# cfframe/spatial-VAE

Hardware: AMD Instinct MI355X
Metric: images/sec (ELBO fwd+bwd+step), MNIST 28x28 batch=256, 1/2/4/8 GPU (higher is better)
Workload: dtype f32; 1 GPU; mnist-rotated-translated 28x28 z=2 H=500x2 tanh B=256 (BASELINE configs[1]); global_batch=256, per_gpu_batch=256, pixels=784, parallelism=dp1

## Files before the change

### spatial_vae_amd/csrc/api.hip

```cpp
#include <stdarg.h>
#include <stdio.h>
#include <stdlib.h>
#include <string.h>
#include <math.h>
#include <atomic>
#include <mutex>
#include <iterator>
#include <type_traits>
#include <unordered_map>
#include <vector>

#include "common.h"
#include "../../include/svae_stream.h"
#include "../../include/svae_align.h"
#include "../../include/svae_ctfcorr.h"
#include "../../include/svae_cluster.h"
#include "../../include/svae_frc.h"
#include "../../include/svae_refine.h"
#include "../../include/svae_classify.h"
#include "../../include/svae_gmm.h"
#include "../../include/svae_pca.h"
#include "../../include/svae_expect.h"
#include <hip/hip_ext.h>
#include "dense.h"
// ... 347 lines not shown
int launch_status(const char* what) {
    const hipError_t e = hipGetLastError();
    if (e != hipSuccess) return fail(SVAE_E_LAUNCH, "%s: %s", what, hipGetErrorString(e));
    return SVAE_OK;
}

inline unsigned blocks_for(long n) { return (unsigned)((n + 255) / 256); }

PoseArgs pose_args(const svae_pose* pose) {
    PoseArgs pa;
    pa.coords = pose->coords;
    pa.grid = pose->grid;
    pa.theta = pose->coords ? nullptr : pose->theta;
    pa.dx = pose->coords ? nullptr : pose->dx;
    return pa;
}

RowGeo row_geo(const Geo& g) {
    RowGeo r;
    r.N = g.N; r.Npad = g.Npad; r.Hp = g.Hp; r.in_dim = g.in_dim; r.act = g.act; r.B = g.B;
    return r;
}

void launch_prepare(const Geo& g, const Plan& pl, const svae_params* p, const PoseArgs& pa, const float* z, hipStream_t st) {
    Scope prof(K_PREPARE, st);
    PrepareArgs a;
    a.coord_w = p->coord_w; a.coord_b = p->coord_b;
    a.latent_w = g.Zd > 0 ? p->latent_w : nullptr;
    a.bil_w = (g.flags & SVAE_FLAG_BILINEAR) ? p->bilinear_w : nullptr;
    a.z = z; a.tab = pl.tab; a.posebuf = pl.posebuf; a.pose = pa;
    a.B = g.B; a.H = g.H; a.Hp = g.Hp; a.Zd = g.Zd; a.in_dim = g.in_dim;
    const long nt = (long)g.B * g.Hp;
    a.nb_tab = (int)blocks_for(nt > g.B ? nt : g.B);
    a.nb_pack = (int)blocks_for((long)g.Hp * g.Hp);
    a.nlayers = g.L - 1;
    for (int l = 0; l < SVAE_MAX_HIDDEN; ++l) {
        const bool on = l + 1 < g.L;
        a.W[l] = on ? p->hidden_w[l] : nullptr;
        a.wf[l] = on ? pl.wf[l] : nullptr;
        a.wb[l] = on ? pl.wb[l] : nullptr;
        a.wb_row_scale[l] = (on && l == g.L - 2 && rank1_out(g)) ? p->out_w : nullptr;
    }
    hipLaunchKernelGGL(prepare_kernel, dim3((unsigned)(a.nb_tab + a.nb_pack * a.nlayers)), dim3(256), 0, st, a);
}

template <int NT, bool DGRAD, bool RESID, bool FIRST, int LASTD, int CF = 0>
void launch_dense_ntr(const DenseArgs& a, dim3 grid, hipStream_t st) {
    constexpr int kLds = DenseCfg<NT>::LDS_BYTES + (LASTD == 1 ? SVAE_MAX_OUT * 4096 * 4 : 0);
    const int lds = DenseCfg<NT>::LDS_BYTES + (LASTD == 1 ? SVAE_MAX_OUT * a.Hp * 4 : 0);
    static bool attr_set = false;
    if (!attr_set) {
        (void)hipFuncSetAttribute(reinterpret_cast<const void*>(&dense_kernel<NT, DGRAD, RESID, FIRST, LASTD, CF>),
                                  hipFuncAttributeMaxDynamicSharedMemorySize, kLds < 160 * 1024 ? kLds : 160 * 1024);
        attr_set = true;
    }
    launch_gemm(dense_kernel<NT, DGRAD, RESID, FIRST, LASTD, CF>, grid, dim3(256), (unsigned)lds, st, a);
}

template <int NT, bool DGRAD>
void launch_dense_nt(const DenseArgs& a, dim3 grid, hipStream_t st, bool first = false, int lastd = 0, int cf = 0) {
    if constexpr (!DGRAD && NT <= 4) {
        if (cf >= 1) {
            if (a.resid) launch_dense_ntr<NT, false, true, false, 0, 1>(a, grid, st);
            else launch_dense_ntr<NT, false, false, false, 0, 1>(a, grid, st);
            return;
// ... 372 lines not shown
        else launch_gemm(wgrad2_kernel<0>, grid, dim3(256), 0u, st, w);
        return;
    }
    const int nb2 = w.nblk1 * w.nblk1;
    w.S = (xcd && nb2 > 1 && nsplit % 8 == 0) ? nsplit : 0;
    const dim3 grid = w.S ? dim3(nb2 * nsplit) : dim3(nb2, nsplit);
    if (r1 == 1) {
        launch_wgrad_c<1, 1>(w, grid, st);
        return;
    }
    if (r1 == 2) {
        launch_wgrad_c<1, 2>(w, grid, st);
        return;
    }
    switch (cl) {
        case 1: launch_wgrad_c<1>(w, grid, st); break;
        case 2: launch_wgrad_c<2>(w, grid, st); break;
        case 3: launch_wgrad_c<3>(w, grid, st); break;
        case 4: launch_wgrad_c<4>(w, grid, st); break;
        default: launch_wgrad_c<0>(w, grid, st); break;
    }
}

template <int ACT>
void launch_layer0_fwd(const Geo& g, const Plan& pl, const PoseArgs& pa, float* a0, hipStream_t st) {
    Scope prof(K_LAYER0_FWD, st);
    const int oimg = g.Npad / 8;
    const int cpi = (oimg + kL0Chunk - 1) / kL0Chunk;
    const int opc = (oimg + cpi - 1) / cpi;
    const long nchunks = (long)g.B * cpi;
    const unsigned gy = (unsigned)(nchunks < 32768 ? nchunks : 32768);
    const unsigned gz = (unsigned)((nchunks + gy - 1) / gy);
    hipLaunchKernelGGL((layer0_fwd_kernel<ACT>), dim3(blocks_for(g.Hp * 2), gy, gz), dim3(256), 0, st, pa, pl.posebuf,
                       pl.tab, a0, row_geo(g), opc, (oimg + opc - 1) / opc, nchunks);
}

template <int ACT>
void launch_layer0_fwd_split(const Geo& g, const Plan& pl, const PoseArgs& pa, float* a0, bool saved_ok, hipStream_t st) {
    Scope prof(K_LAYER0_FWD, st);
    hipLaunchKernelGGL((layer0_fwd_split_kernel<ACT>), dim3((unsigned)g.tiles, (unsigned)(g.Hp / 64)), dim3(256), 0, st, pa,
                       pl.posebuf, pl.tab, split_a0_fragments_only(g) ? (float*)nullptr : a0, pl.splitA,
                       (saved_ok && g.L == 2) ? pl.savedC : (uint4*)nullptr, row_geo(g));
}

template <int C>
void launch_out_fwd(const Geo& g, const float* a, const svae_params* p, float* y, float* logits, hipStream_t st) {
    Scope prof(K_OUT_FWD, st);
    long nb = (g.noct + 3) / 4;
    if (nb > 4096) nb = 4096;
    hipLaunchKernelGGL((out_fwd_kernel<C>), dim3((unsigned)nb), dim3(256), 0, st, a, p->out_w, p->out_b, y, logits,
                       row_geo(g), g.H, (g.flags & SVAE_FLAG_SOFTPLUS) ? 1 : 0, g.noct);
}

template <int ACT, int C>
void launch_out_bwd_ac(const Geo& g, const Plan& pl, const float* a, const svae_params* p, float* dh, hipStream_t st) {
    Scope prof(K_OUT_BWD, st);
    hipLaunchKernelGGL((out_bwd_kernel<ACT, C>), dim3(blocks_for(g.Hp * 2), pl.ob_chunks), dim3(256), 0, st, a, pl.do_p,
// ... 41 lines not shown
        return fail(SVAE_E_INVALID, "softplus output with a Bernoulli likelihood: the reference's binary_cross_entropy rejects "
                                    "values above 1 (train_mnist.py:81)");
    if (d->Zd > 0 && !z) return fail(SVAE_E_INVALID, "latent_dim > 0 but z is null");
    if (saved && (reinterpret_cast<uintptr_t>(saved) & 255)) return fail(SVAE_E_WORKSPACE, "saved not 256-byte aligned");
    const Geo g = make_geo(*d);
    Plan pl = make_plan(g, saved, ws);
    if ((rc = check_ws(pl, ws, ws_bytes))) return rc;
    hipStream_t st = static_cast<hipStream_t>(stream);
    const PoseArgs pa = pose_args(pose);
    if (!saved) {
        for (int l = 0; l < g.L; ++l) pl.act[l] = pl.dh[l & 1];
    } else {
        remember_plan(saved, plan_bits(g));
    }

    const char* fuse_e = getenv("SVAE_FUSE_LOGITS");
    const bool fuse_env = !(fuse_e && fuse_e[0] == '0');
    const bool split_fwd = split_mode() && (g.act == SVAE_ACT_TANH || g.act == SVAE_ACT_SIGMOID) && g.ntile % 2 == 0;
    const bool fuse_logits = fuse_env && g.L >= 2 &&
                             (split_fwd ? g.C <= 2
                                        : g.C <= 2 * (use_dense4(g, g.flags & SVAE_FLAG_RESID, 0) ? use_dense4(g, g.flags & SVAE_FLAG_RESID, 0)
                                                                                                   : dense_nt_first(g.ntile)));

    launch_prepare(g, pl, p, pa, z, st);
    const bool split = split_mode() && (g.act == SVAE_ACT_TANH || g.act == SVAE_ACT_SIGMOID) && g.ntile % 2 == 0;
    const bool split_l0 = split_l0_on() && split && g.L >= 2;
    if (split_l0) {
        if (g.act == SVAE_ACT_TANH) launch_layer0_fwd_split<SVAE_ACT_TANH>(g, pl, pa, pl.act[0], saved != nullptr, st);
        else launch_layer0_fwd_split<SVAE_ACT_SIGMOID>(g, pl, pa, pl.act[0], saved != nullptr, st);
    } else {
        switch (g.act) {
            case SVAE_ACT_TANH: launch_layer0_fwd<SVAE_ACT_TANH>(g, pl, pa, pl.act[0], st); break;
            case SVAE_ACT_LEAKYRELU: launch_layer0_fwd<SVAE_ACT_LEAKYRELU>(g, pl, pa, pl.act[0], st); break;
            case SVAE_ACT_RELU: launch_layer0_fwd<SVAE_ACT_RELU>(g, pl, pa, pl.act[0], st); break;
            default: launch_layer0_fwd<SVAE_ACT_SIGMOID>(g, pl, pa, pl.act[0], st); break;
        }
    }
    DenseBlocks cfb{dense_nt_first(g.ntile), (long)g.Mp, 1};
    for (int l = 1; l < g.L; ++l) {
        if (split) {
            launch_split_fwd(g, pl, pl.act[l - 1], p->hidden_w[l - 1], p->hidden_b[l - 1], pl.act[l],
                             (g.flags & SVAE_FLAG_RESID) != 0, (fuse_logits && l == g.L - 1) ? g.C : 0, p->out_w,
                             split_l0 && l == 1, st);
            continue;
        }
        DenseArgs a;
        a.in = pl.act[l - 1];
        a.wp = pl.wf[l - 1];
        a.out = pl.act[l];
        a.bias = p->hidden_b[l - 1];
        a.aux = nullptr;
        a.tiles = g.tiles;
        a.Hp = g.Hp;
        a.H = g.H;
        a.act = g.act;
        a.resid = (g.flags & SVAE_FLAG_RESID) ? 1 : 0;
        a.pose = pa; a.posebuf = nullptr; a.tab = nullptr; a.sgtile = nullptr; a.dfpart = nullptr;
        a.Mp = g.Mp; a.N = g.N; a.Timg = g.Timg;
        a.do_p = nullptr; a.out_w = p->out_w; a.C = g.C;
        a.lpart = pl.dfpart;
        const DenseBlocks used = launch_dense<false>(g, a, st, false, 0, (fuse_logits && l == g.L - 1) ? g.C : 0);
        if (l == g.L - 1) cfb = used;
    }
    if (fuse_logits) {
        Scope prof(K_OUT_FWD, st);
        const int nblk = g.ntile / (split ? split_nt_fwd(g) : cfb.nt);
        const long m_split = split ? (long)g.Mp : cfb.m_split;
        const int nblk_tail = g.ntile / cfb.nt_tail;
        if (bce_target) {
            const int chunks = finish_chunks(g.N);
            hipLaunchKernelGGL(logits_finish_bce_kernel, dim3(g.B, chunks), dim3(g.N > 512 ? 1024 : (g.N > 256 ? 512 : 256)), 0, st,
                               pl.dfpart, p->out_b, bce_target, y, logits, chunks > 1 ? pl.llpart : loglik, dll_dy, row_geo(g), g.C,
                               nblk, (long)g.Mp, m_split, nblk_tail);
            if (chunks > 1)
                hipLaunchKernelGGL(loglik_reduce_kernel, dim3(blocks_for(g.B)), dim3(256), 0, st, pl.llpart, loglik, g.B, chunks);
        }
        else
            hipLaunchKernelGGL(logits_finish_kernel, dim3(blocks_for((long)g.B * g.N)), dim3(256), 0, st, pl.dfpart, p->out_b, y,
                               logits, row_geo(g), g.C, nblk, (g.flags & SVAE_FLAG_SOFTPLUS) ? 1 : 0, (long)g.Mp, m_split, nblk_tail);
        return launch_status("svae_decoder_forward");
    }
    switch (g.C) {
// ... 32 lines not shown
    if ((rc = check_desc(d)) || (rc = check_params(d, p)) || (rc = check_pose(pose))) return rc;
    if (!logits || !dy || !saved || !grads) return fail(SVAE_E_INVALID, "logits, dy, saved and grads are required");
    if (d->Zd > 0 && !z) return fail(SVAE_E_INVALID, "latent_dim > 0 but z is null");
    if (reinterpret_cast<uintptr_t>(saved) & 255) return fail(SVAE_E_WORKSPACE, "saved not 256-byte aligned");
    if (pg && (pg->dtheta || pg->ddx) && pose->coords)
        return fail(SVAE_E_INVALID, "dtheta/ddx requested but the pose was given as explicit coords");
    const Geo g = make_geo(*d);
    {
        const long rec = recorded_plan(saved);
        if (rec >= 0 && (unsigned)rec != plan_bits(g))
            return fail(SVAE_E_INVALID, "svae_decoder_backward: `saved` was written by a forward call planned differently (plan "
                        "bits %ld then, %u now): the GEMM mode (svae_gemm_mode_set / SVAE_GEMM) or SVAE_FUSE_OUT changed between "
                        "the forward call and its backward call", rec, plan_bits(g));
    }
    const Plan pl = make_plan(g, const_cast<void*>(saved), ws);
    if ((rc = check_ws(pl, ws, ws_bytes))) return rc;
    hipStream_t st = static_cast<hipStream_t>(stream);
    const PoseArgs pa = pose_args(pose);
    const int resid = (g.flags & SVAE_FLAG_RESID) ? 1 : 0;
    const int fmode = fuse_out_mode();
    const bool split_bwd = split_active(g) && g.L >= 2 && fmode != 1;
    const bool r1 = rank1_out(g);

    {
        Scope prof(K_DLOGITS, st);
        if (split_bwd && hipMemsetAsync(pl.amax, 0, sizeof(unsigned), st) != hipSuccess) return fail(SVAE_E_LAUNCH, "memset failed");
        hipLaunchKernelGGL(dlogits_kernel, dim3(blocks_for((long)g.C * g.Mp)), dim3(256), 0, st, logits, dy, dy_scale,
                           pl.do_p, g.B, g.N, g.Npad, g.C, (g.flags & SVAE_FLAG_SOFTPLUS) ? 1 : 0, (long)g.Mp,
                           split_bwd ? pl.amax : (unsigned*)nullptr);
        if (split_bwd)
            hipLaunchKernelGGL(split_scale_kernel, dim3(1), dim3(256), 0, st, pl.amax, p->out_w, g.C, g.H, pl.gscale);
    }

    int cur = 0;
    const bool fused_out = r1 || (fmode == 1 && g.L >= 2 && !resid && (grads->hidden_w[g.L - 2] || grads->hidden_b[g.L - 2]));
    int ob_nparts = 0;
    static const bool ob_env = [] { const char* e = getenv("SVAE_SPLIT_OB"); return !(e && e[0] == '0'); }();
    const bool split_ob = ob_env && split_bwd && split_wgrad_on() && (grads->hidden_w[g.L - 2] || grads->hidden_b[g.L - 2]);
    if (split_ob) {
        const float* alast = pl.act[g.L - 1];
        float* dh32 = resid ? pl.dh[cur] : nullptr;
        const int nparts = g.act == SVAE_ACT_TANH ? launch_out_bwd_split_a<SVAE_ACT_TANH>(g, pl, alast, p, dh32, st)
                                                  : launch_out_bwd_split_a<SVAE_ACT_SIGMOID>(g, pl, alast, p, dh32, st);
        ob_nparts = nparts;
        Scope prof(K_SMALL_BWD, st);
        hipLaunchKernelGGL(out_bwd_reduce_kernel, dim3(g.C * ((g.Hp + 63) / 64) + 1), dim3(1024), 0, st, pl.wpart, pl.bpart,
                           grads->out_w, grads->out_b, g.C, g.H, g.Hp, nparts);
    } else if (!fused_out) {
        const float* alast = pl.act[g.L - 1];
        switch (g.act) {
            case SVAE_ACT_TANH: launch_out_bwd_a<SVAE_ACT_TANH>(g, pl, alast, p, pl.dh[cur], st); break;
            case SVAE_ACT_LEAKYRELU: launch_out_bwd_a<SVAE_ACT_LEAKYRELU>(g, pl, alast, p, pl.dh[cur], st); break;
            case SVAE_ACT_RELU: launch_out_bwd_a<SVAE_ACT_RELU>(g, pl, alast, p, pl.dh[cur], st); break;
            default: launch_out_bwd_a<SVAE_ACT_SIGMOID>(g, pl, alast, p, pl.dh[cur], st); break;
        }
        Scope prof(K_SMALL_BWD, st);
        hipLaunchKernelGGL(out_bwd_reduce_kernel, dim3(g.C * ((g.Hp + 63) / 64) + 1), dim3(1024), 0, st, pl.wpart, pl.bpart,
                           grads->out_w, grads->out_b, g.C, g.H, g.Hp, pl.ob_chunks * 2);
    }

    bool fused_first = false;
    bool tail_pending = false;
    WgradReduceArgs tail_r{};
    bool obr_pending = false;
    OutBwdReduceArgs tail_o{};
    const bool dcoords_wanted = pg && pg->dcoords;
    DenseBlocks fb{dense_nt_first(g.ntile), (long)g.Mp, 1};
    for (int l = g.L - 1; l >= 1; --l) {
        const bool last = fused_out && l == g.L - 1;
        const bool split_here = split_bwd && (l == g.L - 1 || split_chain_on());
        if (grads->hidden_w[l - 1] || grads->hidden_b[l - 1] || (last && (grads->out_w || grads->out_b))) {
            WgradArgs w;
            w.dh = last ? pl.act[l] : pl.dh[cur];
            w.aprev = pl.act[l - 1];
            w.slab = pl.slab;
            w.bslab = pl.bslab;
            w.noct = g.noct;
            w.vo = (g.N + 7) / 8; w.po = g.Npad / 8;
            w.Hp = g.Hp;
            w.nblk1 = pl.wg_nblk1;
            w.do_p = pl.do_p; w.out_w = p->out_w; w.wpart = pl.wpart; w.bpart = pl.bpart;
            w.Mp = g.Mp; w.H = g.H; w.act = g.act;
            if (split_here && split_wgrad_on())
                launch_split_wgrad(g, pl, pl.dh[cur], pl.act[l - 1],
                                   (l == 1 && g.L == 2 && split_l0_on()) ? pl.savedC : (const uint4*)nullptr,
                                   split_ob && l == g.L - 1, st);
            else {
                static const bool xcd_grid = [] { const char* e = getenv("SVAE_XCD_GRID"); return !(e && e[0] == '0'); }();
                launch_wgrad(w, pl.wg_S, xcd_grid, last ? g.C : 0, (last && r1) ? (g.act == SVAE_ACT_TANH ? 1 : 2) : 0, st);
            }
            Scope prof(K_WGRAD_REDUCE, st);
            const bool db_elsewhere = split_ob && l == g.L - 1 && split_wgrad_on();
            const WgradReduceArgs ra{pl.slab, pl.bslab, grads->hidden_w[l - 1],
                                     db_elsewhere ? (float*)nullptr : grads->hidden_b[l - 1], g.H, g.Hp, pl.wg_S,
                                     (last && r1) ? p->out_w : (const float*)nullptr};
            if (l == 1 && g.in_dim == 2 && !split_here && tail_merge_on()) {
                tail_r = ra;
                tail_pending = true;
            } else {
                hipLaunchKernelGGL(wgrad_reduce_kernel, dim3((unsigned)(((long)g.H * g.H + 63) / 64)), dim3(256), 0, st, ra);
            }
            if (db_elsewhere && grads->hidden_b[l - 1])
                hipLaunchKernelGGL(colsum_reduce_kernel, dim3(g.Hp / 32), dim3(256), 0, st, pl.hbpart, grads->hidden_b[l - 1],
                                   g.H, g.Hp, ob_nparts);
            if (last) {
                tail_o = OutBwdReduceArgs{pl.wpart, pl.bpart, grads->out_w, grads->out_b, g.C, g.H, g.Hp, pl.wg_S * 2};
                obr_pending = true;
            }
        }
        DenseArgs a;
        a.in = last ? pl.act[l] : pl.dh[cur];
        a.wp = pl.wb[l - 1];
        a.out = pl.dh[cur ^ 1];
        a.bias = nullptr;
        a.aux = pl.act[l - 1];
        a.tiles = g.tiles;
        a.Hp = g.Hp;
        a.H = g.H;
        a.act = g.act;
        a.resid = resid;
        a.pose = pa; a.posebuf = pl.posebuf; a.tab = pl.tab; a.sgtile = pl.sgtile; a.dfpart = pl.dfpart;
        a.Mp = g.Mp; a.N = g.N; a.Timg = g.Timg;
        a.do_p = pl.do_p; a.out_w = p->out_w; a.C = g.C;
        fused_first = (l == 1) && g.in_dim == 2;
        if (split_here)
            launch_split_dgrad(g, pl, pl.dh[cur], p->hidden_w[l - 1], pl.act[l - 1], pl.dh[cur ^ 1], resid != 0, fused_first, pa,
                               split_ob && l == g.L - 1, st);
        else {
            const DenseBlocks used = launch_dense<true>(g, a, st, fused_first, last ? (r1 ? (g.act == SVAE_ACT_TANH ? 2 : 3) : 1) : 0,
                                                        0, dcoords_wanted);
            if (l == 1) fb = used;
        }
        cur ^= 1;
    }

    if (tail_pending && !fused_first) {
        tail_pending = false;
        hipLaunchKernelGGL(wgrad_reduce_kernel, dim3((unsigned)(((long)g.H * g.H + 63) / 64)), dim3(256), 0, st, tail_r);
    }
    const unsigned obr_blocks = (unsigned)(g.C * ((g.Hp + 63) / 64) + 1);
    if (obr_pending && !tail_pending) {
        obr_pending = false;
        Scope prof(K_SMALL_BWD, st);
        hipLaunchKernelGGL(out_bwd_reduce_kernel, dim3(obr_blocks), dim3(1024), 0, st, tail_o.wpart, tail_o.bpart, tail_o.dWo,
                           tail_o.dbo, tail_o.C, tail_o.H, tail_o.Hp, tail_o.nparts);
    }
    const bool bil = (g.flags & SVAE_FLAG_BILINEAR) != 0;
    const bool want_coords = pg && (pg->dcoords || pg->dtheta || pg->ddx);
    float* dc = (pg && pg->dcoords) ? pg->dcoords : pl.dcoords;
    {
        Scope prof_l0(K_LAYER0_BWD, st);
        const bool split_first = split_bwd && (g.L == 2 || split_chain_on());
        const bool want_dz = dz && g.Zd > 0;
        const bool pose_sums = fused_first && !pose->coords && !dcoords_wanted && pg && (pg->dtheta || pg->ddx);
// ... 473 lines not shown
```

### spatial_vae_amd/csrc/common.h

```cpp
#pragma once
#include <hip/hip_runtime.h>
#include <stdint.h>

#include "../../include/svae.h"

namespace svae {

typedef float f32x16 __attribute__((ext_vector_type(16)));
typedef float v4f __attribute__((ext_vector_type(4)));

constexpr int kSlots = 8;
constexpr int kBiasSlot = 5;

struct Geo {
    int B, N, H, L, Zd, C, in_dim, act, flags;
    int Timg;
    int Npad;
    int Mp;
    int Hp;
    int ntile;
    long noct;
    long tiles;
};

// ... 67 lines not shown
    if (p.coords) {
        const float2 v = *reinterpret_cast<const float2*>(p.coords + ((long)b * N + i) * 2);
        return v;
    }
    const float2 g = *reinterpret_cast<const float2*>(p.grid + (long)i * 2);
    return make_float2(c * g.x - s * g.y + dx0, s * g.x + c * g.y + dx1);
}

__device__ __forceinline__ void image_pose(const PoseArgs& p, int b, float& c, float& s, float& dx0, float& dx1) {
    c = 1.0f; s = 0.0f; dx0 = 0.0f; dx1 = 0.0f;
    if (!p.coords) {
        if (p.theta) {
            const float t = p.theta[b];
            c = cosf(t);
            s = sinf(t);
        }
        if (p.dx) {
            dx0 = p.dx[2 * b];
            dx1 = p.dx[2 * b + 1];
        }
    }
}

__device__ __forceinline__ float2 row_coord(const PoseArgs& pose, const float4 pb, int b, int i, int N) {
    if (i >= N) return make_float2(0.0f, 0.0f);
    return pixel_coord(pose, b, i, N, pb.x, pb.y, pb.z, pb.w);
}

__device__ __forceinline__ void coord_feats(float2 x, float f[5]) {
    f[0] = x.x; f[1] = x.y; f[2] = x.x * x.x; f[3] = x.y * x.y; f[4] = x.x * x.y;
}

__device__ __forceinline__ float wave_sum32(float v) {
    v += __shfl_xor(v, 1);
    v += __shfl_xor(v, 2);
    v += __shfl_xor(v, 4);
    v += __shfl_xor(v, 8);
    v += __shfl_xor(v, 16);
    return v;
}

template <int CTRL, int ROW_MASK>
__device__ __forceinline__ float dpp_add(float v) {
    const int t = __builtin_amdgcn_update_dpp(0, __float_as_int(v), CTRL, ROW_MASK, 0xf, ROW_MASK == 0xf);
    return v + __int_as_float(t);
}
// ... 62 lines not shown
```

### spatial_vae_amd/csrc/dense.h

```cpp
#pragma once
#include "common.h"

namespace svae {

struct DenseArgs {
    const float* in;
    const float* wp;
    float* out;
    const float* bias;
    const float* aux;
    long tiles;
    int Hp;
    int H;
    int act;
    int resid;
    PoseArgs pose;
    const float4* posebuf;
    const float* tab;
    float* sgtile;
    float* dfpart;
    long Mp;
    int N, Timg;
    const float* do_p;
    const float* out_w;
    int C;
    float* lpart;
};

template <int ACT, bool DGRAD>
__device__ __forceinline__ float4 dense_epilogue(float4 v, float bias, float4 aux) {
    if (DGRAD) {
        v.x *= act_grad<ACT>(aux.x); v.y *= act_grad<ACT>(aux.y);
        v.z *= act_grad<ACT>(aux.z); v.w *= act_grad<ACT>(aux.w);
    } else {
        v.x = act_fwd<ACT>(v.x + bias); v.y = act_fwd<ACT>(v.y + bias);
        v.z = act_fwd<ACT>(v.z + bias); v.w = act_fwd<ACT>(v.w + bias);
    }
    return v;
}

__device__ __forceinline__ void glds16(const float* gsrc, unsigned lds_byte_addr) {
    unsigned keep;
    asm volatile(
        "s_mov_b32 %0, m0\n\ts_mov_b32 m0, %2\n\ts_nop 0\n\tglobal_load_lds_dwordx4 %1, off\n\ts_mov_b32 m0, %0"
        : "=&s"(keep)
        : "v"(gsrc), "s"(lds_byte_addr)
        : "memory");
}
__device__ __forceinline__ void dma_wait_all() { asm volatile("s_waitcnt vmcnt(0)" ::: "memory"); }
// ... 749 lines not shown
```

### spatial_vae_amd/csrc/dense4.h

```cpp
#pragma once
#include "dense.h"

namespace svae {

typedef float f32x4v __attribute__((ext_vector_type(4)));
typedef float f32x2v __attribute__((ext_vector_type(2)));

template <int OFF>
__device__ __forceinline__ void load_a4(const float* p, f32x4v& v) {
    asm volatile("global_load_dwordx4 %0, %1, off offset:%2" : "+v"(v) : "v"(p), "i"(OFF) : "memory");
}
template <int N>
__device__ __forceinline__ void wait_vm4(f32x4v& v) {
    asm volatile("s_waitcnt vmcnt(%1)" : "+v"(v) : "i"(N) : "memory");
}
template <int LASTD>
__device__ __forceinline__ f32x4v rank1_actgrad(f32x4v x) {
    f32x4v r;
#pragma unroll
    for (int i = 0; i < 4; ++i) r[i] = __builtin_fmaf(-x[i], x[i], LASTD == 2 ? 1.0f : x[i]);
    return r;
}

__device__ __forceinline__ float add_uncontracted(float a, float b) {
// ... 63 lines not shown
    auto read_b = [&](int o, float4 (&b)[NT]) {
        const float* base = bfrag + ((o / G) & 1) * CHUNK + (o % G) * NT * 256;
#pragma unroll
        for (int t = 0; t < NT; ++t) b[t] = *reinterpret_cast<const float4*>(base + t * 256);
    };
    constexpr int P = PW;
    constexpr int PE = (P + 3) / 4;
    static_assert(G == 4, "the slot offsets assume 4 octets per chunk");

    float* rowx = smem + 2 * CHUNK + wave * (3 * 128);
    if (FIRST) {
#pragma unroll
        for (int rr = 0; rr < 2; ++rr) {
            const int row = lane + 64 * rr;
            const long tile = rgl * 4 + (row >> 5);
            const int b = (int)(tile / a.Timg);
            const int i = (int)(tile % a.Timg) * 32 + (row & 31);
            const float4 pb = a.posebuf[b];
            const float* cbase = a.pose.coords ? a.pose.coords + (long)b * a.N * 2 : a.pose.grid;
            const float2 g2 = *reinterpret_cast<const float2*>(cbase + (long)(i < a.N ? i : a.N - 1) * 2);
            const bool in = i < a.N;
            rowx[row] = in ? pb.x * g2.x - pb.y * g2.y + pb.z : 0.0f;
            rowx[128 + row] = in ? pb.y * g2.x + pb.x * g2.y + pb.w : 0.0f;
            if (LASTD != 0) rowx[256 + row] = a.do_p[rgl * 128 + row];
        }
    }
    stage(0, 0);
    stage(nchunk > 1 ? 1 : 0, 1);
    f32x4v av[G][4];
    float4 b0[NT], b1[NT];
#pragma unroll
    for (int gl = 0; gl < G; ++gl)
#pragma unroll
        for (int e = 0; e < 4; ++e) av[gl][e] = f32x4v{0.0f, 0.0f, 0.0f, 0.0f};
    load_a4<0>(arow, av[0][0]); load_a4<32>(arow, av[0][1]); load_a4<64>(arow, av[0][2]); load_a4<96>(arow, av[0][3]);
    load_a4<256>(arow, av[1][0]); load_a4<288>(arow, av[1][1]); load_a4<320>(arow, av[1][2]); load_a4<352>(arow, av[1][3]);
    load_a4<512>(arow, av[2][0]); load_a4<544>(arow, av[2][1]); load_a4<576>(arow, av[2][2]); load_a4<608>(arow, av[2][3]);
    load_a4<768>(arow, av[3][0]); load_a4<800>(arow, av[3][1]); load_a4<832>(arow, av[3][2]); load_a4<864>(arow, av[3][3]);
#pragma unroll
    for (int gl = 0; gl < G; ++gl)
#pragma unroll
        for (int e = 0; e < 4; ++e) wait_vm4<0>(av[gl][e]);
    __syncthreads();
    read_b(0, b0);
    const int spare = nchunk & 1;
    auto kstep = [&](const f32x4v& x, const float4 (&bf)[NT], int e) {
#pragma unroll
// ... 266 lines not shown
```

### spatial_vae_amd/csrc/elementwise.h

```cpp
#pragma once
#include <type_traits>
#include "common.h"

namespace svae {

__device__ __forceinline__ long slab_index(int contr, int out, int ntile) {
    return (((long)(contr >> 3) * ntile + (out >> 5)) * 2 + ((contr >> 2) & 1)) * 128 + (out & 31) * 4 + (contr & 3);
}
struct PrepareArgs {
    const float* coord_w; const float* coord_b; const float* latent_w; const float* bil_w; const float* z;
    float* tab; float4* posebuf; PoseArgs pose;
    int B, H, Hp, Zd, in_dim;
    int nb_tab, nb_pack, nlayers;
    const float* W[SVAE_MAX_HIDDEN]; float* wf[SVAE_MAX_HIDDEN]; float* wb[SVAE_MAX_HIDDEN];
    const float* wb_row_scale[SVAE_MAX_HIDDEN];
};
__global__ void __launch_bounds__(256) prepare_kernel(PrepareArgs a) {
    if ((int)blockIdx.x < a.nb_tab) {
        const long idx = (long)blockIdx.x * 256 + threadIdx.x;
        if (idx < a.B) {
            float c, s, d0, d1;
            image_pose(a.pose, (int)idx, c, s, d0, d1);
            a.posebuf[idx] = make_float4(c, s, d0, d1);
        }
        if (idx >= (long)a.B * a.Hp) return;
        const int b = idx / a.Hp, k = idx % a.Hp;
        float out[kSlots] = {0, 0, 0, 0, 0, 0, 0, 0};
        if (k < a.H) {
            for (int p = 0; p < a.in_dim; ++p) {
                float w = a.coord_w[k * a.in_dim + p];
                if (a.bil_w)
                    for (int q = 0; q < a.Zd; ++q) w += a.bil_w[((long)k * a.in_dim + p) * a.Zd + q] * a.z[(long)b * a.Zd + q];
                out[p] = w;
            }
            float bias = a.coord_b[k];
            if (a.latent_w)
                for (int q = 0; q < a.Zd; ++q) bias += a.latent_w[(long)k * a.Zd + q] * a.z[(long)b * a.Zd + q];
            out[kBiasSlot] = bias;
        }
        float4* dst = reinterpret_cast<float4*>(a.tab + idx * kSlots);
        dst[0] = make_float4(out[0], out[1], out[2], out[3]);
        dst[1] = make_float4(out[4], out[5], out[6], out[7]);
        return;
    }
    const int rel = blockIdx.x - a.nb_tab;
    const int l = rel / a.nb_pack;
    const long idx = (long)(rel - l * a.nb_pack) * 256 + threadIdx.x;
    if (l >= a.nlayers || idx >= (long)a.Hp * a.Hp) return;
    const int n = idx / a.Hp, k = idx % a.Hp;
    const float v = (n < a.H && k < a.H) ? a.W[l][(long)n * a.H + k] : 0.0f;
    a.wf[l][slab_index(k, n, a.Hp / 32)] = v;
    a.wb[l][slab_index(n, k, a.Hp / 32)] = (a.wb_row_scale[l] && n < a.H) ? v * a.wb_row_scale[l][n] : v;
}

struct RowGeo {
    int N, Npad, Hp, in_dim, act, B;
};

constexpr int kL0Chunk = 32;
template <int ACT>
__global__ void __launch_bounds__(256) layer0_fwd_kernel(PoseArgs pose, const float4* __restrict__ posebuf,
                                                         const float* __restrict__ tab, float* __restrict__ a0, RowGeo g,
                                                         int oct_per_chunk, int chunks_per_image, long nchunks) {
    __shared__ float4 xs[kL0Chunk * 2 * 2];
    const long chunk = (long)blockIdx.z * gridDim.y + blockIdx.y;
    if (chunk >= nchunks) return;
    const int b = (int)(chunk / chunks_per_image), ci = (int)(chunk - (long)b * chunks_per_image);
    const int oimg = g.Npad >> 3;
    const int oc0 = ci * oct_per_chunk;
    const int noc = (oc0 + oct_per_chunk <= oimg) ? oct_per_chunk : oimg - oc0;
    const float4 pb = posebuf[b];
    const float* cbase = pose.coords ? pose.coords + (long)b * g.N * 2 : pose.grid;
    float* xf = reinterpret_cast<float*>(xs);
    for (int j = threadIdx.x; j < noc * 8; j += 256) {
        const int i = oc0 * 8 + j;
        float x0 = 0.0f, x1 = 0.0f;
        if (i < g.N) {
            const float2 raw = *reinterpret_cast<const float2*>(cbase + (long)i * 2);
            x0 = pb.x * raw.x - pb.y * raw.y + pb.z;
            x1 = pb.y * raw.x + pb.x * raw.y + pb.w;
        }
        const int slot = (j >> 2) * 8 + (j & 3);
        xf[slot] = x0;
        xf[slot + 4] = x1;
    }
    __syncthreads();
    const int t = blockIdx.x * 256 + threadIdx.x;
    if (t >= g.Hp * 2) return;
    const int h = t & 1, k = t >> 1;
    const float4* tp = reinterpret_cast<const float4*>(tab + ((long)b * g.Hp + k) * kSlots);
    const float4 t0 = tp[0], t1 = tp[1];
    const long ostride = (long)g.Hp * 8;
    float* dst = a0 + (((long)b * oimg + oc0) * g.Hp * 2 + t) * 4;
    const bool expand = g.in_dim == 5;
#pragma unroll 4
    for (int jo = 0; jo < noc; ++jo) {
        const float4 X0 = xs[(jo * 2 + h) * 2], X1 = xs[(jo * 2 + h) * 2 + 1];
        const float x0[4] = {X0.x, X0.y, X0.z, X0.w}, x1[4] = {X1.x, X1.y, X1.z, X1.w};
        float out[4];
#pragma unroll
        for (int e = 0; e < 4; ++e) {
            float v = t1.y + x0[e] * t0.x + x1[e] * t0.y;
            if (expand) v += (x0[e] * x0[e]) * t0.z + (x1[e] * x1[e]) * t0.w + (x0[e] * x1[e]) * t1.x;
            out[e] = act_fwd<ACT>(v);
        }
        *reinterpret_cast<float4*>(dst + jo * ostride) = make_float4(out[0], out[1], out[2], out[3]);
    }
}

template <int C>
__global__ void out_fwd_kernel(const float* __restrict__ a, const float* __restrict__ out_w,
                               const float* __restrict__ out_b, float* __restrict__ y, float* __restrict__ logits,
                               RowGeo g, int H, int softplus, long noct) {
    const int lane = threadIdx.x & 63;
    const int nl = lane & 31, h = lane >> 5;
    const long wave0 = (long)blockIdx.x * 4 + (threadIdx.x >> 6);
    const long nwaves = (long)gridDim.x * 4;
    for (long o = wave0; o < noct; o += nwaves) {
        float p[4][C];
#pragma unroll
        for (int e = 0; e < 4; ++e)
#pragma unroll
            for (int c = 0; c < C; ++c) p[e][c] = 0.0f;
        for (int t = 0; t < g.Hp / 32; ++t) {
            const int n = t * 32 + nl;
            const float4 v = *reinterpret_cast<const float4*>(a + ((o * g.Hp + n) * 8 + 4 * h));
#pragma unroll
// ... 76 lines not shown
    if (threadIdx.x == 0) loglik[(long)b * gridDim.y + blockIdx.y] = acc;
}

__global__ void loglik_reduce_kernel(const float* __restrict__ part, float* __restrict__ loglik, int B, int chunks) {
    const int b = blockIdx.x * 256 + threadIdx.x;
    if (b >= B) return;
    float s = 0.0f;
    for (int k = 0; k < chunks; ++k) s += part[(long)b * chunks + k];
    loglik[b] = s;
}

__global__ void dlogits_kernel(const float* __restrict__ logits, const float* __restrict__ dy,
                               const float* __restrict__ dy_scale, float* __restrict__ do_p, int B, int N, int Npad,
                               int C, int softplus, long Mp, unsigned* __restrict__ amax) {
    const long idx = (long)blockIdx.x * 256 + threadIdx.x;
    float m = 0.0f;
    if (idx < (long)C * Mp) {
        const int c = (int)(idx / Mp);
        const long mp = idx - (long)c * Mp;
        const int b = (int)(mp / Npad), i = (int)(mp - (long)b * Npad);
        float v = 0.0f;
        if (i < N) {
            const long src = ((long)b * N + i) * C + c;
            const float lg = logits[src];
            const float s = 1.0f / (1.0f + expf(-lg));
            float g = dy[src];
            if (dy_scale) g *= dy_scale[b];
            if (softplus && c == 0) g *= 1.0f / (1.0f + expf(-s));
            v = g * s * (1.0f - s);
        }
        do_p[idx] = v;
        m = fabsf(v);
    }
    if (amax) {
        __shared__ float red[4];
#pragma unroll
        for (int d = 32; d >= 1; d >>= 1) m = fmaxf(m, __shfl_xor(m, d));
        if ((threadIdx.x & 63) == 0) red[threadIdx.x >> 6] = m;
        __syncthreads();
        if (threadIdx.x == 0) {
            m = fmaxf(fmaxf(red[0], red[1]), fmaxf(red[2], red[3]));
            if (m > 0.0f) atomicMax(amax, __float_as_uint(m));
        }
    }
}

template <int ACT, int C>
__global__ void out_bwd_kernel(const float* __restrict__ a, const float* __restrict__ do_p,
                               const float* __restrict__ out_w, float* __restrict__ dh, float* __restrict__ wpart,
                               float* __restrict__ bpart, int H, int Hp, long Mp, long noct, long oct_per_chunk) {
    const int t = blockIdx.x * 256 + threadIdx.x;
    if (t >= Hp * 2) return;
// ... 1192 lines not shown
```

Measured before the change: 98310 images/s.

## Merge prepare into layer0 forward and fold dlogits into last dgrad kernel

Removes the separate prepare_kernel launch by appending its blocks to the layer0 forward grid. Layer0 blocks recompute pose and table entries inline instead of reading what prepare writes, so they no longer depend on it. In the backward pass, for rank-1 output with two layers, the dlogits computation is folded into the dense4 dgrad kernel, which also writes do_p for the later weight-gradient pass. Dgrad is then ordered before wgrad. This cuts kernel launches and intermediate round trips, at the cost of redundant per-block table arithmetic and explicit FMA ordering to keep numerics matching.

Result: slower. 94800 images/s (-3.6%).

```diff
diff --git a/spatial_vae_amd/csrc/api.hip b/spatial_vae_amd/csrc/api.hip
--- a/spatial_vae_amd/csrc/api.hip
+++ b/spatial_vae_amd/csrc/api.hip
@@ -393,8 +393,7 @@
     return r;
 }
 
-void launch_prepare(const Geo& g, const Plan& pl, const svae_params* p, const PoseArgs& pa, const float* z, hipStream_t st) {
-    Scope prof(K_PREPARE, st);
+PrepareArgs prepare_args(const Geo& g, const Plan& pl, const svae_params* p, const PoseArgs& pa, const float* z) {
     PrepareArgs a;
     a.coord_w = p->coord_w; a.coord_b = p->coord_b;
     a.latent_w = g.Zd > 0 ? p->latent_w : nullptr;
@@ -412,6 +411,10 @@
         a.wb[l] = on ? pl.wb[l] : nullptr;
         a.wb_row_scale[l] = (on && l == g.L - 2 && rank1_out(g)) ? p->out_w : nullptr;
     }
+    return a;
+}
+void launch_prepare(const PrepareArgs& a, hipStream_t st) {
+    Scope prof(K_PREPARE, st);
     hipLaunchKernelGGL(prepare_kernel, dim3((unsigned)(a.nb_tab + a.nb_pack * a.nlayers)), dim3(256), 0, st, a);
 }
 
@@ -830,17 +833,32 @@
     }
 }
 
+bool l0_merge_on() {
+    const char* e = getenv("SVAE_L0_MERGE");
+    return !(e && e[0] == '0');
+}
+
 template <int ACT>
-void launch_layer0_fwd(const Geo& g, const Plan& pl, const PoseArgs& pa, float* a0, hipStream_t st) {
-    Scope prof(K_LAYER0_FWD, st);
+void launch_layer0_fwd(const Geo& g, const Plan& pl, const PoseArgs& pa, const PrepareArgs& prep, float* a0, hipStream_t st) {
     const int oimg = g.Npad / 8;
     const int cpi = (oimg + kL0Chunk - 1) / kL0Chunk;
     const int opc = (oimg + cpi - 1) / cpi;
     const long nchunks = (long)g.B * cpi;
+    const unsigned gx = blocks_for(g.Hp * 2);
     const unsigned gy = (unsigned)(nchunks < 32768 ? nchunks : 32768);
     const unsigned gz = (unsigned)((nchunks + gy - 1) / gy);
-    hipLaunchKernelGGL((layer0_fwd_kernel<ACT>), dim3(blocks_for(g.Hp * 2), gy, gz), dim3(256), 0, st, pa, pl.posebuf,
-                       pl.tab, a0, row_geo(g), opc, (oimg + opc - 1) / opc, nchunks);
+    const long nprep = (long)prep.nb_tab + (long)prep.nb_pack * prep.nlayers;
+    const long zextra = (nprep + (long)gx * gy - 1) / ((long)gx * gy);
+    if (l0_merge_on() && gz + zextra <= 65535) {
+        Scope prof(K_LAYER0_FWD, st);
+        hipLaunchKernelGGL((layer0_fwd_kernel<ACT, true>), dim3(gx, gy, gz + (unsigned)zextra), dim3(256), 0, st, pa, pl.posebuf,
+                           pl.tab, a0, row_geo(g), opc, (oimg + opc - 1) / opc, nchunks, gz, prep);
+        return;
+    }
+    launch_prepare(prep, st);
+    Scope prof(K_LAYER0_FWD, st);
+    hipLaunchKernelGGL((layer0_fwd_kernel<ACT, false>), dim3(gx, gy, gz), dim3(256), 0, st, pa, pl.posebuf, pl.tab, a0,
+                       row_geo(g), opc, (oimg + opc - 1) / opc, nchunks, gz, prep);
 }
 
 template <int ACT>
@@ -928,18 +946,19 @@
                                         : g.C <= 2 * (use_dense4(g, g.flags & SVAE_FLAG_RESID, 0) ? use_dense4(g, g.flags & SVAE_FLAG_RESID, 0)
                                                                                                    : dense_nt_first(g.ntile)));
 
-    launch_prepare(g, pl, p, pa, z, st);
+    const PrepareArgs prep = prepare_args(g, pl, p, pa, z);
     const bool split = split_mode() && (g.act == SVAE_ACT_TANH || g.act == SVAE_ACT_SIGMOID) && g.ntile % 2 == 0;
     const bool split_l0 = split_l0_on() && split && g.L >= 2;
     if (split_l0) {
+        launch_prepare(prep, st);
         if (g.act == SVAE_ACT_TANH) launch_layer0_fwd_split<SVAE_ACT_TANH>(g, pl, pa, pl.act[0], saved != nullptr, st);
         else launch_layer0_fwd_split<SVAE_ACT_SIGMOID>(g, pl, pa, pl.act[0], saved != nullptr, st);
     } else {
         switch (g.act) {
-            case SVAE_ACT_TANH: launch_layer0_fwd<SVAE_ACT_TANH>(g, pl, pa, pl.act[0], st); break;
-            case SVAE_ACT_LEAKYRELU: launch_layer0_fwd<SVAE_ACT_LEAKYRELU>(g, pl, pa, pl.act[0], st); break;
-            case SVAE_ACT_RELU: launch_layer0_fwd<SVAE_ACT_RELU>(g, pl, pa, pl.act[0], st); break;
-            default: launch_layer0_fwd<SVAE_ACT_SIGMOID>(g, pl, pa, pl.act[0], st); break;
+            case SVAE_ACT_TANH: launch_layer0_fwd<SVAE_ACT_TANH>(g, pl, pa, prep, pl.act[0], st); break;
+            case SVAE_ACT_LEAKYRELU: launch_layer0_fwd<SVAE_ACT_LEAKYRELU>(g, pl, pa, prep, pl.act[0], st); break;
+            case SVAE_ACT_RELU: launch_layer0_fwd<SVAE_ACT_RELU>(g, pl, pa, prep, pl.act[0], st); break;
+            default: launch_layer0_fwd<SVAE_ACT_SIGMOID>(g, pl, pa, prep, pl.act[0], st); break;
         }
     }
     DenseBlocks cfb{dense_nt_first(g.ntile), (long)g.Mp, 1};
@@ -964,6 +983,7 @@
         a.pose = pa; a.posebuf = nullptr; a.tab = nullptr; a.sgtile = nullptr; a.dfpart = nullptr;
         a.Mp = g.Mp; a.N = g.N; a.Timg = g.Timg;
         a.do_p = nullptr; a.out_w = p->out_w; a.C = g.C;
+        a.dl_logits = nullptr; a.dl_dy = nullptr; a.dl_scale = nullptr; a.do_out = nullptr; a.dl_softplus = 0;
         a.lpart = pl.dfpart;
         const DenseBlocks used = launch_dense<false>(g, a, st, false, 0, (fuse_logits && l == g.L - 1) ? g.C : 0);
         if (l == g.L - 1) cfb = used;
@@ -1042,7 +1062,12 @@
     const bool split_bwd = split_active(g) && g.L >= 2 && fmode != 1;
     const bool r1 = rank1_out(g);
 
-    {
+    const bool fold_dlogits = [&] {
+        const char* e = getenv("SVAE_DLOGITS_FOLD");
+        return !(e && e[0] == '0') && r1 && g.L == 2 && g.in_dim == 2 && !split_bwd &&
+               use_dense4(g, resid, g.act == SVAE_ACT_TANH ? 2 : 3) != 0;
+    }();
+    if (!fold_dlogits) {
         Scope prof(K_DLOGITS, st);
         if (split_bwd && hipMemsetAsync(pl.amax, 0, sizeof(unsigned), st) != hipSuccess) return fail(SVAE_E_LAUNCH, "memset failed");
         hipLaunchKernelGGL(dlogits_kernel, dim3(blocks_for((long)g.C * g.Mp)), dim3(256), 0, st, logits, dy, dy_scale,
@@ -1089,7 +1114,8 @@
     for (int l = g.L - 1; l >= 1; --l) {
         const bool last = fused_out && l == g.L - 1;
         const bool split_here = split_bwd && (l == g.L - 1 || split_chain_on());
-        if (grads->hidden_w[l - 1] || grads->hidden_b[l - 1] || (last && (grads->out_w || grads->out_b))) {
+        auto weight_gradient = [&] {
+            if (!(grads->hidden_w[l - 1] || grads->hidden_b[l - 1] || (last && (grads->out_w || grads->out_b)))) return;
             WgradArgs w;
             w.dh = last ? pl.act[l] : pl.dh[cur];
             w.aprev = pl.act[l - 1];
@@ -1127,29 +1153,40 @@
                 tail_o = OutBwdReduceArgs{pl.wpart, pl.bpart, grads->out_w, grads->out_b, g.C, g.H, g.Hp, pl.wg_S * 2};
                 obr_pending = true;
             }
-        }
-        DenseArgs a;
-        a.in = last ? pl.act[l] : pl.dh[cur];
-        a.wp = pl.wb[l - 1];
-        a.out = pl.dh[cur ^ 1];
-        a.bias = nullptr;
-        a.aux = pl.act[l - 1];
-        a.tiles = g.tiles;
-        a.Hp = g.Hp;
-        a.H = g.H;
-        a.act = g.act;
-        a.resid = resid;
-        a.pose = pa; a.posebuf = pl.posebuf; a.tab = pl.tab; a.sgtile = pl.sgtile; a.dfpart = pl.dfpart;
-        a.Mp = g.Mp; a.N = g.N; a.Timg = g.Timg;
-        a.do_p = pl.do_p; a.out_w = p->out_w; a.C = g.C;
-        fused_first = (l == 1) && g.in_dim == 2;
-        if (split_here)
-            launch_split_dgrad(g, pl, pl.dh[cur], p->hidden_w[l - 1], pl.act[l - 1], pl.dh[cur ^ 1], resid != 0, fused_first, pa,
-                               split_ob && l == g.L - 1, st);
-        else {
-            const DenseBlocks used = launch_dense<true>(g, a, st, fused_first, last ? (r1 ? (g.act == SVAE_ACT_TANH ? 2 : 3) : 1) : 0,
-                                                        0, dcoords_wanted);
-            if (l == 1) fb = used;
+        };
+        auto data_gradient = [&] {
+            DenseArgs a;
+            a.in = last ? pl.act[l] : pl.dh[cur];
+            a.wp = pl.wb[l - 1];
+            a.out = pl.dh[cur ^ 1];
+            a.bias = nullptr;
+            a.aux = pl.act[l - 1];
+            a.tiles = g.tiles;
+            a.Hp = g.Hp;
+            a.H = g.H;
+            a.act = g.act;
+            a.resid = resid;
+            a.pose = pa; a.posebuf = pl.posebuf; a.tab = pl.tab; a.sgtile = pl.sgtile; a.dfpart = pl.dfpart;
+            a.Mp = g.Mp; a.N = g.N; a.Timg = g.Timg;
+            a.do_p = pl.do_p; a.out_w = p->out_w; a.C = g.C;
+            a.dl_logits = fold_dlogits ? logits : nullptr; a.dl_dy = dy; a.dl_scale = dy_scale; a.do_out = pl.do_p;
+            a.dl_softplus = (g.flags & SVAE_FLAG_SOFTPLUS) ? 1 : 0;
+            fused_first = (l == 1) && g.in_dim == 2;
+            if (split_here)
+                launch_split_dgrad(g, pl, pl.dh[cur], p->hidden_w[l - 1], pl.act[l - 1], pl.dh[cur ^ 1], resid != 0, fused_first, pa,
+                                   split_ob && l == g.L - 1, st);
+            else {
+                const DenseBlocks used = launch_dense<true>(g, a, st, fused_first, last ? (r1 ? (g.act == SVAE_ACT_TANH ? 2 : 3) : 1) : 0,
+                                                            0, dcoords_wanted);
+                if (l == 1) fb = used;
+            }
+        };
+        if (fold_dlogits) {
+            data_gradient();
+            weight_gradient();
+        } else {
+            weight_gradient();
+            data_gradient();
         }
         cur ^= 1;
     }
diff --git a/spatial_vae_amd/csrc/common.h b/spatial_vae_amd/csrc/common.h
--- a/spatial_vae_amd/csrc/common.h
+++ b/spatial_vae_amd/csrc/common.h
@@ -113,6 +113,13 @@
     }
 }
 
+__device__ __forceinline__ float dlogit_value(float lg, float g, const float* __restrict__ dy_scale, int b, bool softplus) {
+    const float s = 1.0f / (1.0f + expf(-lg));
+    if (dy_scale) g *= dy_scale[b];
+    if (softplus) g *= 1.0f / (1.0f + expf(-s));
+    return g * s * (1.0f - s);
+}
+
 __device__ __forceinline__ float2 row_coord(const PoseArgs& pose, const float4 pb, int b, int i, int N) {
     if (i >= N) return make_float2(0.0f, 0.0f);
     return pixel_coord(pose, b, i, N, pb.x, pb.y, pb.z, pb.w);
diff --git a/spatial_vae_amd/csrc/dense.h b/spatial_vae_amd/csrc/dense.h
--- a/spatial_vae_amd/csrc/dense.h
+++ b/spatial_vae_amd/csrc/dense.h
@@ -25,6 +25,11 @@
     const float* out_w;
     int C;
     float* lpart;
+    const float* dl_logits;
+    const float* dl_dy;
+    const float* dl_scale;
+    float* do_out;
+    int dl_softplus;
 };
 
 template <int ACT, bool DGRAD>
diff --git a/spatial_vae_amd/csrc/dense4.h b/spatial_vae_amd/csrc/dense4.h
--- a/spatial_vae_amd/csrc/dense4.h
+++ b/spatial_vae_amd/csrc/dense4.h
@@ -109,7 +109,17 @@
             const bool in = i < a.N;
             rowx[row] = in ? pb.x * g2.x - pb.y * g2.y + pb.z : 0.0f;
             rowx[128 + row] = in ? pb.y * g2.x + pb.x * g2.y + pb.w : 0.0f;
-            if (LASTD != 0) rowx[256 + row] = a.do_p[rgl * 128 + row];
+            if (LASTD != 0) {
+                float dv;
+                if (a.dl_logits) {
+                    const long src = (long)b * a.N + (in ? i : 0);
+                    dv = in ? dlogit_value(a.dl_logits[src], a.dl_dy[src], a.dl_scale, b, a.dl_softplus != 0) : 0.0f;
+                    if (nb == 0 && live) a.do_out[rgl * 128 + row] = dv;
+                } else {
+                    dv = a.do_p[rgl * 128 + row];
+                }
+                rowx[256 + row] = dv;
+            }
         }
     }
     stage(0, 0);
diff --git a/spatial_vae_amd/csrc/elementwise.h b/spatial_vae_amd/csrc/elementwise.h
--- a/spatial_vae_amd/csrc/elementwise.h
+++ b/spatial_vae_amd/csrc/elementwise.h
@@ -15,9 +15,25 @@
     const float* W[SVAE_MAX_HIDDEN]; float* wf[SVAE_MAX_HIDDEN]; float* wb[SVAE_MAX_HIDDEN];
     const float* wb_row_scale[SVAE_MAX_HIDDEN];
 };
-__global__ void __launch_bounds__(256) prepare_kernel(PrepareArgs a) {
-    if ((int)blockIdx.x < a.nb_tab) {
-        const long idx = (long)blockIdx.x * 256 + threadIdx.x;
+__device__ __forceinline__ void table_entry(const PrepareArgs& a, int b, int k, float (&out)[kSlots]) {
+#pragma unroll
+    for (int s = 0; s < kSlots; ++s) out[s] = 0.0f;
+    if (k < a.H) {
+        for (int p = 0; p < a.in_dim; ++p) {
+            float w = a.coord_w[k * a.in_dim + p];
+            if (a.bil_w)
+                for (int q = 0; q < a.Zd; ++q) w += a.bil_w[((long)k * a.in_dim + p) * a.Zd + q] * a.z[(long)b * a.Zd + q];
+            out[p] = w;
+        }
+        float bias = a.coord_b[k];
+        if (a.latent_w)
+            for (int q = 0; q < a.Zd; ++q) bias += a.latent_w[(long)k * a.Zd + q] * a.z[(long)b * a.Zd + q];
+        out[kBiasSlot] = bias;
+    }
+}
+__device__ __forceinline__ void prepare_block(const PrepareArgs& a, int blk) {
+    if (blk < a.nb_tab) {
+        const long idx = (long)blk * 256 + threadIdx.x;
         if (idx < a.B) {
             float c, s, d0, d1;
             image_pose(a.pose, (int)idx, c, s, d0, d1);
@@ -25,25 +41,14 @@
         }
         if (idx >= (long)a.B * a.Hp) return;
         const int b = idx / a.Hp, k = idx % a.Hp;
-        float out[kSlots] = {0, 0, 0, 0, 0, 0, 0, 0};
-        if (k < a.H) {
-            for (int p = 0; p < a.in_dim; ++p) {
-                float w = a.coord_w[k * a.in_dim + p];
-                if (a.bil_w)
-                    for (int q = 0; q < a.Zd; ++q) w += a.bil_w[((long)k * a.in_dim + p) * a.Zd + q] * a.z[(long)b * a.Zd + q];
-                out[p] = w;
-            }
-            float bias = a.coord_b[k];
-            if (a.latent_w)
-                for (int q = 0; q < a.Zd; ++q) bias += a.latent_w[(long)k * a.Zd + q] * a.z[(long)b * a.Zd + q];
-            out[kBiasSlot] = bias;
-        }
+        float out[kSlots];
+        table_entry(a, b, k, out);
         float4* dst = reinterpret_cast<float4*>(a.tab + idx * kSlots);
         dst[0] = make_float4(out[0], out[1], out[2], out[3]);
         dst[1] = make_float4(out[4], out[5], out[6], out[7]);
         return;
     }
-    const int rel = blockIdx.x - a.nb_tab;
+    const int rel = blk - a.nb_tab;
     const int l = rel / a.nb_pack;
     const long idx = (long)(rel - l * a.nb_pack) * 256 + threadIdx.x;
     if (l >= a.nlayers || idx >= (long)a.Hp * a.Hp) return;
@@ -52,24 +57,44 @@
     a.wf[l][slab_index(k, n, a.Hp / 32)] = v;
     a.wb[l][slab_index(n, k, a.Hp / 32)] = (a.wb_row_scale[l] && n < a.H) ? v * a.wb_row_scale[l][n] : v;
 }
+__global__ void __launch_bounds__(256) prepare_kernel(PrepareArgs a) { prepare_block(a, (int)blockIdx.x); }
 
 struct RowGeo {
     int N, Npad, Hp, in_dim, act, B;
 };
 
+__device__ __forceinline__ float2 l0_posed(const float4 pb, const float2 raw) {
+#pragma clang fp contract(off)
+    return make_float2(__builtin_fmaf(pb.x, raw.x, -(pb.y * raw.y)) + pb.z, __builtin_fmaf(pb.y, raw.x, pb.x * raw.y) + pb.w);
+}
+__device__ __forceinline__ float l0_preact(float x0, float x1, const float4 t0, const float4 t1, bool expand) {
+#pragma clang fp contract(off)
+    const float v = __builtin_fmaf(x0, t0.x, t1.y) + x1 * t0.y;
+    if (!expand) return v;
+    return v + ((x0 * x1) * t1.x + __builtin_fmaf(x1 * x1, t0.w, (x0 * x0) * t0.z));
+}
+
 constexpr int kL0Chunk = 32;
-template <int ACT>
+template <int ACT, bool MERGED>
 __global__ void __launch_bounds__(256) layer0_fwd_kernel(PoseArgs pose, const float4* __restrict__ posebuf,
                                                          const float* __restrict__ tab, float* __restrict__ a0, RowGeo g,
-                                                         int oct_per_chunk, int chunks_per_image, long nchunks) {
+                                                         int oct_per_chunk, int chunks_per_image, long nchunks, unsigned zprep,
+                                                         PrepareArgs prep) {
     __shared__ float4 xs[kL0Chunk * 2 * 2];
+    if (MERGED && blockIdx.z >= zprep) {
+        const long blk = ((long)(blockIdx.z - zprep) * gridDim.y + blockIdx.y) * gridDim.x + blockIdx.x;
+        if (blk < (long)prep.nb_tab + (long)prep.nb_pack * prep.nlayers) prepare_block(prep, (int)blk);
+        return;
+    }
     const long chunk = (long)blockIdx.z * gridDim.y + blockIdx.y;
     if (chunk >= nchunks) return;
     const int b = (int)(chunk / chunks_per_image), ci = (int)(chunk - (long)b * chunks_per_image);
     const int oimg = g.Npad >> 3;
     const int oc0 = ci * oct_per_chunk;
     const int noc = (oc0 + oct_per_chunk <= oimg) ? oct_per_chunk : oimg - oc0;
-    const float4 pb = posebuf[b];
+    float4 pb;
+    if (MERGED) image_pose(pose, b, pb.x, pb.y, pb.z, pb.w);
+    else pb = posebuf[b];
     const float* cbase = pose.coords ? pose.coords + (long)b * g.N * 2 : pose.grid;
     float* xf = reinterpret_cast<float*>(xs);
     for (int j = threadIdx.x; j < noc * 8; j += 256) {
@@ -77,8 +102,9 @@
         float x0 = 0.0f, x1 = 0.0f;
         if (i < g.N) {
             const float2 raw = *reinterpret_cast<const float2*>(cbase + (long)i * 2);
-            x0 = pb.x * raw.x - pb.y * raw.y + pb.z;
-            x1 = pb.y * raw.x + pb.x * raw.y + pb.w;
+            const float2 xp = l0_posed(pb, raw);
+            x0 = xp.x;
+            x1 = xp.y;
         }
         const int slot = (j >> 2) * 8 + (j & 3);
         xf[slot] = x0;
@@ -88,8 +114,17 @@
     const int t = blockIdx.x * 256 + threadIdx.x;
     if (t >= g.Hp * 2) return;
     const int h = t & 1, k = t >> 1;
-    const float4* tp = reinterpret_cast<const float4*>(tab + ((long)b * g.Hp + k) * kSlots);
-    const float4 t0 = tp[0], t1 = tp[1];
+    float4 t0, t1;
+    if (MERGED) {
+        float e[kSlots];
+        table_entry(prep, b, k, e);
+        t0 = make_float4(e[0], e[1], e[2], e[3]);
+        t1 = make_float4(e[4], e[5], e[6], e[7]);
+    } else {
+        const float4* tp = reinterpret_cast<const float4*>(tab + ((long)b * g.Hp + k) * kSlots);
+        t0 = tp[0];
+        t1 = tp[1];
+    }
     const long ostride = (long)g.Hp * 8;
     float* dst = a0 + (((long)b * oimg + oc0) * g.Hp * 2 + t) * 4;
     const bool expand = g.in_dim == 5;
@@ -100,9 +135,7 @@
         float out[4];
 #pragma unroll
         for (int e = 0; e < 4; ++e) {
-            float v = t1.y + x0[e] * t0.x + x1[e] * t0.y;
-            if (expand) v += (x0[e] * x0[e]) * t0.z + (x1[e] * x1[e]) * t0.w + (x0[e] * x1[e]) * t1.x;
-            out[e] = act_fwd<ACT>(v);
+            out[e] = act_fwd<ACT>(l0_preact(x0[e], x1[e], t0, t1, expand));
         }
         *reinterpret_cast<float4*>(dst + jo * ostride) = make_float4(out[0], out[1], out[2], out[3]);
     }
@@ -225,12 +258,7 @@
         float v = 0.0f;
         if (i < N) {
             const long src = ((long)b * N + i) * C + c;
-            const float lg = logits[src];
-            const float s = 1.0f / (1.0f + expf(-lg));
-            float g = dy[src];
-            if (dy_scale) g *= dy_scale[b];
-            if (softplus && c == 0) g *= 1.0f / (1.0f + expf(-s));
-            v = g * s * (1.0f - s);
+            v = dlogit_value(logits[src], dy[src], dy_scale, b, softplus && c == 0);
         }
         do_p[idx] = v;
         m = fabsf(v);
```
